# fenghansen/YOND_public

Measured on AMD Instinct MI355X. Metric: Bayer megapixels/sec end-to-end (NLE+VST+denoise+iVST), higher is better.
Workload: dtype f32 (3x3 convolutions: f32 operands as two f16 halves -- 22-23 significant bits -- on the f16 MFMA, 3 products per f32 product, f32 accumulate; per-layer error vs float64 asserted <= 2x the f32 direct kernel's and <= 2e-5 of max|ref| (tests/test_hip_conv.py; measured 1.3e-6 vs 1.5e-6), whole frame v

## Files before the change

include/yond_hip.h:

```cpp
#ifndef YOND_HIP_H
#define YOND_HIP_H

#include <stddef.h>
#include <stdint.h>

#ifdef __cplusplus
extern "C" {
#endif

#define YOND_OK 0
#define YOND_EINVAL (-1)
#define YOND_EUNSUPPORTED (-2)

#define YOND_ABI_VERSION 8
int yond_abi_version(void);

int yond_pack_vst_norm_f32(const float* bayer, int H, int W, float* out, int pad_l, int pad_r, int pad_t,
                           int pad_b, int mode, double scale, double gain, double sigma, double lo,
                           double hi, const double* lut_x, const float* lut_y, int lut_n, float* img_max,
                           void* stream);

int yond_pack_vst_norm_biaslut_f32(const float* bayer, int H, int W, float* out, int pad_l, int pad_r, int pad_t,
                                   int pad_b, double scale, double gain, double sigma, double lo, double hi,
                                   const double* lut_x, const double* lut_y, int lut_n, float* img_max, void* stream);
// ... 28 lines not shown
typedef struct YondConvDesc {
    const float* src0;
    const float* src1;
    int C0, C1;
    int N, H, W;
    int Ho, Wo;
    int Cout;
    int ksize;
    int stride;
    int shuffle;
    int pre_act;
    int post_act;
    float slope;
    const float* wpk;
    const float* escale;
    const float* eshift;
    int ebatch;
    const float* res;
    float* dst;
    int tn;
    int kc;
    int algo;
    const float* out4_w;
    const float* out4_b;
    const float* out4_x;
    const float* out4_ub;
    float* out4_dst;
    unsigned int* status;
    int in_fmt, out_fmt;
    int res_fmt;
    unsigned long long* clk;
    int tile_order;
    float* dst2;
} YondConvDesc;
#define YOND_STATUS_HALF_OVERFLOW 1u
#define YOND_FMT_NHWC_F32 0
#define YOND_FMT_SPLIT_PLANES 1
#define YOND_FMT_PLANES4 2
#define YOND_SP_PLANE_UNITS(H, W) ((((H) * (W)) + 8) / 8 * 8)
#define YOND_SP_BYTES(N, C, H, W) ((size_t)(N) * ((C) / 16) * 4 * (size_t)YOND_SP_PLANE_UNITS(H, W) * 16)
#define YOND_HP_BYTES(N, C, H, W) ((size_t)(N) * ((C) / 16) * 2 * (size_t)YOND_SP_PLANE_UNITS(H, W) * 16)

int yond_conv_config(int ksize, int stride, int cin, int cout, int shuffle, int N, int Ho, int Wo, int* tn, int* kc);
int yond_pack_conv_weight_f32(const float* w, int cout, int cin, int ksize, int tn, int kc, float* dst);
int yond_pack_conv_weight_split_f32(const float* w, int cout, int cin, int ksize, int tn, int kc, float* dst);
int yond_conv2d_f32(const YondConvDesc* desc, void* stream);

int yond_conv_wino_supported(int cin, int cout);
int yond_pack_conv_wino_weight_f32(const float* w, int cout, int cin, int tn, float* dst);

int yond_conv_split_supported(int ksize, int stride, int cin, int cout);
int yond_pack_conv_split_weight_f32(const float* w, int cout, int cin, int ksize, int tn, int parts, float* dst);
int yond_gemm_k1_stationary_supported(const YondConvDesc* desc);
int yond_pack_conv_split_weight_dev_f32(const float* w, int cout, int cin, int ksize, int tn, int parts, float* dst, int* status,
                                        void* stream);
int yond_pack_conv_split_weights_batch_dev_f32(const float* src, const long long* desc, int nlayers, float* dst, size_t ngroups,
                                               int* status, void* stream);

int yond_conv_in_f32(const float* x, const float* ub , int N, int H, int W, int Cout,
                     const float* wpk, const float* bias, float slope, float* dst,
                     int out_fmt , void* stream);
int yond_pack_conv_in_weight_f32(const float* w , int cout, float* dst );

int yond_conv_out_f32(const float* feat , int Cin, const float* w ,
                      const float* bias , const float* x ,
                      const float* ub , int N, int H, int W, float* dst ,
                      void* stream);

int yond_maxpool2_f32(const float* src, int N, int H, int W, int C, float* dst, void* stream);

typedef struct YondFilmDesc {
    int kind, C, ld;
    const float *w_a0, *b_a0, *w_a2, *b_a2;
    const float *w_b0, *b_b0;
    const float *w_b, *b_b;
    const float *cb1, *cb2;
    float *s1, *t1, *s2, *t2;
} YondFilmDesc;
int yond_film_f32(const YondFilmDesc* descs, int nblocks, const float* t , const float* ub ,
                  int N, void* stream);

int yond_box_stats_self1_f32(const float* bayer, int H, int W, int k, int k2, int tile_w, float* mean,
                             float* var, float* blur2, void* stream);
int yond_box_stats_self2_f32(const float* blur2, int h, int w, int k, int tile_w, float* lap, void* stream);
int yond_box_stats_collab_f32(const float* bayer_lr, const float* bayer_hr, int H, int W, int k, int tile_w,
                              float* mean, float* var, float* lap, void* stream);


int yond_box_stats_self_stats_f32(const float* bayer, int H, int W, int k, int k2, int tile_w, float* mean, float* var,
                                  float* blur2, float* lap, const double* q_host, int nq, void* ws, void* stream);
int yond_box_stats_collab_stats_f32(const float* bayer_lr, const float* bayer_hr, int H, int W, int k, int tile_w,
                                    float* mean, float* var, float* lap, const double* q_host, int nq, void* ws, void* stream);

size_t yond_select_ws_bytes(int nr);
int yond_select_ranks_f32(const float* data, size_t n, const int64_t* ranks_host, int nr, float* out, void* ws,
                          void* stream);
int yond_percentiles_f32(const float* data, size_t n, const double* q_host, int nq, double* out, void* ws,
                         void* stream);

size_t yond_nle_ws_bytes(size_t n);
int yond_nle_stats_f32(const float* lap, const float* mean, size_t n, int width, const double* q_host, int nq, void* ws,
                       void* stream);
int yond_nle_threshold_f32(const float* lap, size_t n, const double* q_host, int nq, int want_score, void* ws, void* stream);
int yond_nle_state_layout(int* off );
int yond_nle_moments_f32(const float* lap, const float* mean, const float* var, size_t n, void* ws, void* stream);

// ... 214 lines not shown
```

yond_public_amd/_lib.py:

```python
import ctypes as C
import os

import torch

_HERE = os.path.dirname(os.path.abspath(__file__))
LIB_PATH = os.environ.get("YOND_HIP_LIB", os.path.join(_HERE, "libyond_hip.so"))
_lib = None
ABI_VERSION = 8

vp, i32, f32, f64, sz, i64 = C.c_void_p, C.c_int, C.c_float, C.c_double, C.c_size_t, C.c_longlong


class YondConvDesc(C.Structure):
    _fields_ = [("src0", vp), ("src1", vp), ("C0", i32), ("C1", i32), ("N", i32), ("H", i32), ("W", i32),
                ("Ho", i32), ("Wo", i32), ("Cout", i32), ("ksize", i32), ("stride", i32), ("shuffle", i32),
                ("pre_act", i32), ("post_act", i32), ("slope", f32), ("wpk", vp), ("escale", vp),
                ("eshift", vp), ("ebatch", i32), ("res", vp), ("dst", vp), ("tn", i32), ("kc", i32), ("algo", i32),
                ("out4_w", vp), ("out4_b", vp), ("out4_x", vp), ("out4_ub", vp), ("out4_dst", vp), ("status", vp),
                ("in_fmt", i32), ("out_fmt", i32), ("res_fmt", i32), ("clk", vp), ("tile_order", i32), ("dst2", vp)]


class YondBlock0Desc(C.Structure):
    _fields_ = [("x", vp), ("in_fmt", i32), ("N", i32), ("H", i32), ("W", i32), ("w1", vp), ("w2", vp),
                ("s1", vp), ("t1", vp), ("s2", vp), ("t2", vp), ("ebatch", i32), ("dst", vp),
                ("out4_w", vp), ("out4_b", vp), ("out4_x", vp), ("out4_ub", vp), ("out4_dst", vp), ("status", vp)]


class YondFilmDesc(C.Structure):
    _fields_ = [("kind", i32), ("C", i32), ("ld", i32),
                ("w_a0", vp), ("b_a0", vp), ("w_a2", vp), ("b_a2", vp), ("w_b0", vp), ("b_b0", vp),
                ("w_b", vp), ("b_b", vp), ("cb1", vp), ("cb2", vp),
                ("s1", vp), ("t1", vp), ("s2", vp), ("t2", vp)]


PROTOTYPES = {
    "yond_abi_version": [],
    "yond_pack_vst_norm_f32": [vp, i32, i32, vp, i32, i32, i32, i32, i32, f64, f64, f64, f64, f64, vp, vp, i32, vp, vp],
    "yond_pack_vst_norm_biaslut_f32": [vp, i32, i32, vp, i32, i32, i32, i32, f64, f64, f64, f64, f64, vp, vp, i32, vp, vp],
    "yond_bias_eval_f32": [vp, sz, vp, vp, i32, i32, i32, f64, f64, vp, vp],
    "yond_denorm_ivst_unpack_f32": [vp, i32, i32, i32, i32, i32, i32, vp, i32, f64, f64, f64, f64, f64, i32, vp],
    "yond_pack_vst_norm_batch_f32": [vp, i32, i32, i32, vp, i32, i32, i32, i32, f64, f64, f64, f64, f64, vp, vp, i32, i32, vp, vp],
    "yond_denorm_ivst_unpack_batch_f32": [vp, i32, i32, i32, i32, i32, i32, i32, vp, i32, f64, f64, f64, f64, f64, i32, vp],
    "yond_vst_elem_f32": [vp, sz, f64, f64, f64, vp, vp],
    "yond_ivst_elem_f64": [vp, sz, f64, f64, i32, vp, vp],
    "yond_bayer2rggb_f32": [vp, i32, i32, vp, vp],
    "yond_rggb2bayer_f32": [vp, i32, i32, vp, vp],
    "yond_rot90_f32": [vp, i32, i32, i32, i32, vp, vp],
    "yond_nchw4_to_nhwc4_f32": [vp, vp, i32, i32, i32, vp],
    "yond_nhwc4_to_nchw4_f32": [vp, vp, i32, i32, i32, vp],
    "yond_image_max_f32": [vp, i32, sz, vp, vp, vp],
    "yond_conv_config": [i32, i32, i32, i32, i32, i32, i32, i32, C.POINTER(i32), C.POINTER(i32)],
    "yond_pack_conv_weight_f32": [vp, i32, i32, i32, i32, i32, vp],
    "yond_conv2d_f32": [C.POINTER(YondConvDesc), vp],
    "yond_conv_wino_supported": [i32, i32],
    "yond_pack_conv_wino_weight_f32": [vp, i32, i32, i32, vp],
    "yond_pack_conv_weight_split_f32": [vp, i32, i32, i32, i32, i32, vp],
    "yond_conv_split_supported": [i32, i32, i32, i32],
    "yond_pack_conv_split_weight_f32": [vp, i32, i32, i32, i32, i32, vp],
    "yond_gemm_k1_stationary_supported": [C.POINTER(YondConvDesc)],
    "yond_pack_conv_split_weight_dev_f32": [vp, i32, i32, i32, i32, i32, vp, vp, vp],
    "yond_pack_conv_split_weights_batch_dev_f32": [vp, vp, i32, vp, sz, vp, vp],
    "yond_conv_in_f32": [vp, vp, i32, i32, i32, i32, vp, vp, f32, vp, i32, vp],
    "yond_pack_conv_in_weight_f32": [vp, i32, vp],
    "yond_conv_out_f32": [vp, i32, vp, vp, vp, vp, i32, i32, i32, vp, vp],
    "yond_maxpool2_f32": [vp, i32, i32, i32, i32, vp, vp],
    "yond_film_f32": [vp, i32, vp, vp, i32, vp],
    "yond_box_stats_self1_f32": [vp, i32, i32, i32, i32, i32, vp, vp, vp, vp],
    "yond_box_stats_self2_f32": [vp, i32, i32, i32, i32, vp, vp],
    "yond_box_stats_collab_f32": [vp, vp, i32, i32, i32, i32, vp, vp, vp, vp],
    "yond_box_stats_self_stats_f32": [vp, i32, i32, i32, i32, i32, vp, vp, vp, vp, vp, i32, vp, vp],
    "yond_box_stats_collab_stats_f32": [vp, vp, i32, i32, i32, i32, vp, vp, vp, vp, i32, vp, vp],
    "yond_select_ws_bytes": [i32],
    "yond_select_ranks_f32": [vp, sz, vp, i32, vp, vp, vp],
    "yond_percentiles_f32": [vp, sz, vp, i32, vp, vp, vp],
    "yond_nle_ws_bytes": [sz],
    "yond_nle_stats_f32": [vp, vp, sz, i32, vp, i32, vp, vp],
    "yond_nle_threshold_f32": [vp, sz, vp, i32, i32, vp, vp],
    "yond_nle_state_layout": [vp],
    "yond_nle_moments_f32": [vp, vp, vp, sz, vp, vp],
    "yond_nlf_occupancy_f32": [vp, vp, sz, i32, vp, i32, vp, vp],
    "yond_nlf_score3_f64": [vp, vp, vp, i32, vp, vp, vp],
    "yond_nlf_moments_f32": [vp, vp, vp, sz, vp, vp, vp],
    "yond_bias_lut_f64": [vp, i32, f64, f64, vp, vp],
    "yond_block_metrics_tiles": [i32, i32],
    "yond_block_metrics_f32": [vp, vp, i32, i32, i32, i32, vp, vp],
    "yond_block_metrics_rgb8": [vp, vp, i32, i32, i32, i32, vp, vp],
    "yond_render_srgb": [vp, i32, i32, i32, i32, i32, C.POINTER(f64), C.POINTER(f64), i32, vp, vp, i32, vp, f64, vp],
    "yond_clock_probe": [f64, vp, vp],
    "yond_img2raw_f32": [vp, sz, i32, i32, i32, vp, vp, i32, i32, i32, vp, vp, vp, vp],
    "yond_pg_noise_f32": [vp, vp, sz, i32, vp, i32, vp],
    "yond_camera_noise_f32": [vp, vp, sz, i32, vp, i32, i32, vp],
    "yond_est_conv_in_f32": [vp, i32, i32, i32, i32, vp, vp, vp, vp],
    "yond_est_head_f32": [vp, i32, i32, i32, i32, vp, vp, i32, i32, i32, vp, vp, vp],
    "yond_est_head_ws_bytes": [i32, i32],
    "yond_conv_wgrad_f32": [vp, vp, i32, i32, i32, i32, i32, i32, i32, i32, i32, vp, vp],
    "yond_conv_wgrad_ws_f32": [vp, vp, i32, i32, i32, i32, i32, i32, i32, i32, i32, vp, vp, sz, vp],
    "yond_conv_wgrad_ws_bytes": [i32, i32, i32, i32, i32, i32, i32, i32, i32],
    "yond_conv_wgrad_split_ws_bytes": [i32, i32, i32, i32, i32],
    "yond_conv_wgrad_split_f32": [vp, vp, i32, i32, i32, i32, i32, vp, i32, vp, sz, vp, vp],
    "yond_colsum_f32": [vp, sz, i32, vp, vp],
    "yond_film_silu_supported": [i32],
    "yond_film_silu_f32": [vp, vp, vp, vp, i32, sz, i32, vp],
    "yond_film_silu_bwd_f32": [vp, vp, vp, vp, vp, vp, vp, i32, sz, i32, vp],
    "yond_film_mlp_fwd_f32": [vp, vp, vp, vp, vp, vp, vp, i32, i32, i32, vp, vp, vp],
    "yond_film_mlp_bwd_f32": [vp, vp, vp, vp, vp, vp, vp, vp, i32, i32, i32, vp, vp, vp, vp, vp, vp, vp, vp],
    "yond_film_mlp_fwd_multi_f32": [vp, i32, vp],
    "yond_gemm_split_f32": [vp, i32, sz, i32, i32, i64, i64, i32, vp, vp, i32, i32, i32, i32, vp, vp],
    "yond_film_mlp_bwd_multi_f32": [vp, i32, vp],
    "yond_silu_bwd_add_f32": [vp, vp, vp, vp, sz, vp],
    "yond_silu_f32": [vp, vp, sz, vp],
    "yond_zero_interleave_f32": [vp, i32, i32, i32, i32, i32, i32, vp, vp],
    "yond_l1_loss_f32": [vp, vp, sz, vp, vp, vp],
# ... 113 lines not shown
```

yond_public_amd/csrc/conv.hip:

```cpp
#include "common.h"
#include <cstdlib>

#ifndef YOND_B32_WGS
#define YOND_B32_WGS 2
#endif
#ifndef YOND_ABL
#define YOND_ABL 0
#endif

template <int KS, int STRIDE, int TH, int TN, int KC>
struct ConvCfg {
    static constexpr int TW = 32;
    static constexpr int TAPS = KS * KS;
    static constexpr int PADK = KS / 2;
    static constexpr int IH = (TH - 1) * STRIDE + KS;
    static constexpr int IW = (TW - 1) * STRIDE + KS;
    static constexpr int HALF = (IW + 1) / 2;
    static constexpr int TWP = (STRIDE == 2) ? 2 * HALF : IW;
    static constexpr int PS = KC + 4;
    static constexpr int IN_FLOATS = IH * TWP * PS;
    static constexpr int Q = KC / 8;
    static constexpr int W_FLOATS = TAPS * Q * 2 * TN * 4;
    static constexpr int BUF_FLOATS = IN_FLOATS + W_FLOATS;
    static constexpr int NW = TN / 32;
// ... 467 lines not shown
    {
        const long e11 = yond_exp_long("YOND_1X1_TN", 0), es2 = yond_exp_long("YOND_S2_TN", 0), ekc = yond_exp_long("YOND_CONV_KC", 0),
                   etn = yond_exp_long("YOND_CONV_TN", 0);
        if (e11 && ksize == 1) t = e11 == 32 ? 32 : (ntile % 64 == 0 ? 64 : 32);
        if (es2 && ksize == 3 && stride == 2) t = es2 == 32 ? 32 : (ntile % 64 == 0 ? 64 : 32);
        if (ekc && ksize == 3 && stride == 1) k = ekc == 8 ? 8 : 16;
        if (etn && ksize == 3 && stride == 1 && ntile % 64 == 0) t = etn == 32 ? 32 : 64;
    }
#endif
    if (tn) *tn = t;
    if (kc) *kc = k;
    return YOND_OK;
}

extern "C" int yond_pack_conv_weight_f32(const float* w, int cout, int cin, int ksize, int tn, int kc, float* dst) {
    if (!w || !dst || (tn != 32 && tn != 64) || cout % tn != 0 || cin % kc != 0 || kc % 8 != 0) return YOND_EINVAL;
    const int taps = ksize * ksize, Q = kc / 8;
    size_t o = 0;
    for (int ct = 0; ct < cout / tn; ++ct)
        for (int ch = 0; ch < cin / kc; ++ch)
            for (int tap = 0; tap < taps; ++tap)
                for (int q = 0; q < Q; ++q)
                    for (int h = 0; h < 2; ++h)
                        for (int j = 0; j < tn; ++j)
                            for (int e = 0; e < 4; ++e) {
                                const int co = ct * tn + j, ci = ch * kc + q * 8 + h * 4 + e;
                                dst[o++] = w[((size_t)co * cin + ci) * taps + tap];
                            }
    return YOND_OK;
}

extern "C" int yond_pack_conv_weight_split_f32(const float* w, int cout, int cin, int ksize, int tn, int kc, float* dst) {
    const int rc = yond_pack_conv_weight_f32(w, cout, cin, ksize, tn, kc, dst);
    if (rc != YOND_OK) return rc;
    const size_t n = (size_t)cout * cin * ksize * ksize;
    for (size_t i = 0; i < n; ++i)
        if (!(fabsf(w[i]) <= 65504.0f)) return YOND_EUNSUPPORTED;
    for (size_t i = 0; i < n; ++i) {
        const float v = dst[i];
        const _Float16 h = (_Float16)v;
        const _Float16 l = (_Float16)((v - (float)h) * 2048.0f);
        unsigned short hb, lb;
        __builtin_memcpy(&hb, &h, 2);
        __builtin_memcpy(&lb, &l, 2);
        const unsigned u = (unsigned)hb | ((unsigned)lb << 16);
        __builtin_memcpy(&dst[i], &u, 4);
    }
    return YOND_OK;
}

int yond_conv_wino_dispatch(const YondConvDesc& d, hipStream_t st);
int yond_conv_split_dispatch(const YondConvDesc& d, hipStream_t st);
int yond_gemm_k1_stationary_dispatch(const YondConvDesc& d, hipStream_t st);

extern "C" int yond_conv2d_f32(const YondConvDesc* dp, void* stream) {
    if (!dp) return YOND_EINVAL;
    const YondConvDesc& d = *dp;
    hipStream_t st = (hipStream_t)stream;
    if (!d.src0 || !(d.dst || d.out4_dst) || !d.wpk || d.N <= 0 || d.H <= 0 || d.W <= 0 || d.Ho <= 0 || d.Wo <= 0) return YOND_EINVAL;
    if (d.out4_dst && ((d.algo != 3 && d.algo != 4) || !d.out4_w || d.Cout != 32 || d.stride != 1)) return YOND_EUNSUPPORTED;
    if (d.C1 > 0 && !d.src1) return YOND_EINVAL;
    if (d.shuffle < 0 || d.shuffle > 2) return YOND_EINVAL;
    if (d.shuffle == 2 && d.algo != 3 && d.algo != 4 && d.algo != 6) return YOND_EUNSUPPORTED;
    if ((long long)d.N * d.H * d.W > 0x7fffffffLL) return YOND_EUNSUPPORTED;
    if (d.pre_act != 0 && d.pre_act != 1) return YOND_EINVAL;
    if (d.in_fmt < 0 || d.in_fmt > 2 || d.out_fmt < 0 || d.out_fmt > 2 || (d.res_fmt != 0 && d.res_fmt != 2)) return YOND_EINVAL;
    if (d.algo == 6) return yond_gemm_k1_stationary_dispatch(d, st);
    if ((d.in_fmt || d.out_fmt || d.res_fmt) && d.algo != 3 && d.algo != 4) return YOND_EUNSUPPORTED;
    if (d.algo == 1) return yond_conv_wino_dispatch(d, st);
    if (d.algo == 3 || d.algo == 4) return yond_conv_split_dispatch(d, st);
    if (d.algo != 0 && d.algo != 2 && d.algo != 5) return YOND_EINVAL;
    if (d.tn != 32 && d.tn != 64) return YOND_EINVAL;
    int tn, kc;
    const int rc = yond_conv_config(d.ksize, d.stride, d.C0 + d.C1, d.Cout, d.shuffle, 0, 0, 0, &tn, &kc);
    if (rc != YOND_OK) return rc;
    tn = d.tn;
    if (d.kc != 0) kc = d.kc;
    if (kc != 8 && kc != 16) return YOND_EINVAL;
    if (kc == 8 && d.ksize != 3) return YOND_EINVAL;
    if (d.ksize == 3 && d.stride == 2 && kc != 8) return YOND_EINVAL;
    if (d.C0 % kc != 0 || d.C1 % kc != 0 || d.Cout % tn != 0) return YOND_EUNSUPPORTED;
    if (d.shuffle && (d.ksize != 1 || (d.Cout / 4) % tn != 0)) return YOND_EUNSUPPORTED;
    if ((long long)d.N * d.H * d.W > 0x7fffffffLL) return YOND_EUNSUPPORTED;
    if (d.stride == 2) {
        if (d.Ho != (d.H + 1) / 2 || d.Wo != (d.W + 1) / 2) return YOND_EINVAL;
    } else if (d.Ho != d.H || d.Wo != d.W) return YOND_EINVAL;
    if (d.pre_act != 0 && d.pre_act != 1) return YOND_EINVAL;
    if (d.post_act != 0 && d.post_act != 2) return YOND_EUNSUPPORTED;
    if (d.pre_act == 1 && !(d.ksize == 3 && d.stride == 1)) return YOND_EUNSUPPORTED;
    if (d.ksize == 3 && d.stride == 1 && kc == 8) {
        if (d.pre_act) return tn == 64 ? launch_conv<3, 1, 8, 64, 8, true>(d, st) : launch_conv<3, 1, 8, 32, 8, true>(d, st);
        return tn == 64 ? launch_conv<3, 1, 8, 64, 8, false>(d, st) : launch_conv<3, 1, 8, 32, 8, false>(d, st);
    }
    if (d.ksize == 3 && d.stride == 1) {
        if (d.pre_act) return tn == 64 ? launch_conv<3, 1, 8, 64, 16, true>(d, st) : launch_conv<3, 1, 8, 32, 16, true>(d, st);
        return tn == 64 ? launch_conv<3, 1, 8, 64, 16, false>(d, st) : launch_conv<3, 1, 8, 32, 16, false>(d, st);
    }
    if (d.ksize == 3 && d.stride == 2)
        return tn == 64 ? launch_conv<3, 2, 8, 64, 8, false>(d, st) : launch_conv<3, 2, 4, 32, 8, false>(d, st);
    return tn == 64 ? launch_conv<1, 1, 8, 64, 16, false>(d, st) : launch_conv<1, 1, 8, 32, 16, false>(d, st);
}
```

yond_public_amd/engine.py:

```python
import ctypes as C
import os

import numpy as np
import torch

from . import _lib as L


def _rup(c, m=32):
    return (c + m - 1) // m * m


def _np_ptr(a):
    return C.c_void_p(a.ctypes.data)


FILM_MAX_C = 1024


WINO_DEFAULT = 'split'


SPLIT_PLANES = True
SP_FLOW = True
HALF_FLOW = True
HALF_K1_TN128 = True
HALF_S2_TN128 = True
HALF_FLOW_TN128 = True
HALF_TN128 = True
FUSE_OUT4 = True
FUSE_BLOCK0 = False
K1_SUB2 = True
K1_D2_LEVELS = (3,)
K1_STATIONARY_LEVELS = (2, 1, 0)
K1_D2_LEVELS_HALF = ()
SP_CONV1_MIN_LEVEL = 3
UNET_SP = True
SNAKE_ORDER = True


def sp_plane_units(H, W):
    return (H * W + 8) // 8 * 8


class _PackedConv:

    def __init__(self, dev, weight, bias, ksize, stride, splits, shuffle=False):
        lib = L.load()
        w = weight.detach().to('cpu', torch.float32).numpy()
        if shuffle:
            cin, cout = w.shape[0], w.shape[1]
            coutp = _rup(cout)
            m = np.zeros((4, coutp, cin), np.float32)
            m[:, :cout, :] = w.transpose(2, 3, 1, 0).reshape(4, cout, cin)
            w = m.reshape(4 * coutp, cin, 1, 1)
            self.cout_real_p = coutp
            gemm_n = 4 * coutp
        else:
            cout = w.shape[0]
            coutp = _rup(cout)
            gemm_n = coutp
            self.cout_real_p = coutp
        assert sum(splits) == w.shape[1], (splits, w.shape)
        psplits = [_rup(s) for s in splits]
        cinp = sum(psplits)
        wp = np.zeros((gemm_n, cinp, ksize, ksize), np.float32)
        so, do = 0, 0
        for s, ps in zip(splits, psplits):
            wp[:w.shape[0], do:do + s] = w[:, so:so + s]
            so += s
            do += ps
        self._wp = np.ascontiguousarray(wp)
        self._packed = {}
        self._dev = dev
        b = torch.zeros(coutp, dtype=torch.float32)
        if bias is not None:
            b[:cout] = bias.detach().to('cpu', torch.float32)
        self.bias = b.to(dev)
        self.ksize, self.stride, self.shuffle = ksize, stride, shuffle
        self.psplits, self.gemm_n, self.coutp, self.cinp = psplits, gemm_n, coutp, cinp
        self.cin_real, self.cout_real = sum(splits), cout
        self.config(0, 0, 0)
        self.wmax = float(np.abs(self._wp).max()) if self._wp.size else 0.0
        self.macs_per_pixel = self.cin_real * self.cout_real * (4 if shuffle else ksize * ksize)

    def config(self, N, Ho, Wo, split=False):
        lib = L.load()
# ... 239 lines not shown
        d.ksize, d.stride, d.shuffle = pc.ksize, pc.stride, int(pc.shuffle)
        d.pre_act, d.post_act, d.slope = pre_act, post_act, slope
        prec = getattr(self, 'precision', 'fp32')
        if getattr(self, 'strict', False) and algo is None:
            prec, algo = 'fp32-mfma', 1
        if algo is None:
            algo = getattr(self, 'conv_algo', WINO_DEFAULT)
            if prec == 'fp32-mfma' and algo == 'split':
                algo = 1
            if prec == 'fp16' and WINO_DEFAULT == 'split':
                algo = 'half'
        fp16 = prec == 'fp16' or algo == 'fp16'
        wino = split = None
        if algo in ('split', 'half'):
            ws2 = (HALF_S2_TN128 and algo == 'half' and pc.stride == 2 and in_fmt == 1 and out_fmt == 2 and dst2 is None
                   and (pc.gemm_n // 128) * ((d.Wo + 31) // 32) * ((d.Ho + 7) // 8) * N >= 256)
            ws2 = ws2 or (HALF_K1_TN128 and algo == 'half' and pc.ksize == 1 and in_fmt == 1 and dst2 is None)
            split = pc.split(2 if algo == 'split' else 1, wide=(not (in_fmt or out_fmt or res_fmt or dst2 is not None)) or (HALF_FLOW_TN128 and out_fmt == 1),
                             wide_s2=ws2)
            if algo == 'half' and pc.ksize == 1 and in_fmt != 1:
                split = None
            if split is None and not fp16 and pc.ksize == 3:
                wino = pc.wino()
        elif not fp16:
            wino = pc.wino() if algo in (1, 2) else None
        if split is not None:
            tn, wpk = split
            kc = 16
            d.algo = 3 if algo == 'split' else 4
        elif wino is not None:
            tn, wpk = wino
            kc = 8
            d.algo = 1
        elif algo == 'split' and pc.ksize == 1 and not fp16 and pc.config(N, d.Ho, d.Wo, split=True)[2] is not None:
            tn, kc, wpk = pc.config(N, d.Ho, d.Wo, split=True)
            d.algo = 5
        else:
            tn, kc, wpk = pc.config(N, d.Ho, d.Wo)
            d.algo = 2 if (fp16 and pc.wmax <= 65504.0) else 0
        d.wpk = wpk.data_ptr()
        d.tn = tn
        d.kc = kc
        d.escale = escale.data_ptr() if escale is not None else None
        d.eshift = (eshift if eshift is not None else pc.bias).data_ptr()
        d.ebatch = ebatch
        d.res = res.data_ptr() if res is not None else None
        d.dst = dst.data_ptr() if dst is not None else None
        status = getattr(self, 'status', None)
        d.status = status.data_ptr() + 4 * self.status_slot if status is not None else None
        d.in_fmt, d.out_fmt, d.res_fmt = in_fmt, out_fmt, res_fmt
        d.dst2 = dst2.data_ptr() if dst2 is not None else None
        if stationary and d.algo == 3 and self.lib.yond_gemm_k1_stationary_supported(C.byref(d)):
            d.algo = 6
        if SNAKE_ORDER and d.algo in (3, 4, 6):
            self._tile_order = 1 - getattr(self, '_tile_order', 0)
            d.tile_order = self._tile_order
        clk = getattr(self, 'clk', None)
        d.clk = clk.data_ptr() if (clk is not None and d.algo in (3, 4, 6)) else None
        if (in_fmt or out_fmt or res_fmt) and d.algo not in (3, 4, 6):
            raise L.YondHipError("split-plane / 4-channel-plane tensors need the split-operand kernel (algo 3, or 4 with h-only planes)")
        if out4 is not None:
            w4, b4, x4, ub4, o4 = out4
            if d.algo not in (3, 4):
                raise L.YondHipError("fused output projection needs the split-operand 3x3 kernel")
            d.out4_w, d.out4_b = w4.data_ptr(), (b4.data_ptr() if b4 is not None else None)
            d.out4_x = x4.data_ptr() if x4 is not None else None
            d.out4_ub = ub4.data_ptr() if ub4 is not None else None
            d.out4_dst = o4.data_ptr()
        prof = getattr(self, 'prof', None)
        if prof is not None:
            tag = f"conv_wino_kernel<{tn}>" if d.algo == 1 else f"conv_mfma_kernel<{pc.ksize},{pc.stride},8,{tn},{kc}>"
            if d.algo in (3, 4, 6):
                tag = f"conv_split_kernel<{pc.stride if pc.ksize == 3 else 'k1'},{tn},{1 if d.algo == 4 else 2}>" + ("/stationary" if d.algo == 6 else "")
            if d.algo == 2:
                tag += "/f16"
            if d.algo == 5:
                tag += "/split"
            only = getattr(self, 'prof_only', None)
            if only is not None and not only(tag):
                prof = None
            every = getattr(self, 'prof_every', 1)
            if every > 1 and getattr(self, '_fwd_idx', 0) % every:
                prof = None
        if prof is not None:
            e0, e1 = torch.cuda.Event(enable_timing=True), torch.cuda.Event(enable_timing=True)
            e0.record()
        L.check(self.lib.yond_conv2d_f32(C.byref(d), L.stream()), "yond_conv2d_f32")
        if prof is not None:
            e1.record()
            prof.append((tag, 2.0 * pc.macs_per_pixel * N * d.Ho * d.Wo, e0, e1))
        return dst

    def _block0_weights(self, pc):
        w = getattr(pc, '_b0', None)
        if w is None:
            if not L.has("yond_pack_block0_weight_f32"):
                raise L.YondHipError("the fused level-0 block exists only in experiment builds of the library (python -m yond_public_amd.build --experiments)")
            if not (pc.ksize == 3 and pc.stride == 1 and pc.gemm_n == 32 and pc.cinp == 32 and len(pc.psplits) == 1):
                return None
            host = np.zeros(9 * 2 * 4 * 32 * 8, np.float16)
            if self.lib.yond_pack_block0_weight_f32(_np_ptr(pc._wp), 32, 32, _np_ptr(host)) != 0:
                return None
            w = pc._b0 = torch.from_numpy(host.view(np.float32)).to(pc._dev)
        return w

    def _block0(self, pc1, pc2, x, N, H, W, f, in_fmt, dst=None, out4=None):
        w1, w2 = self._block0_weights(pc1), self._block0_weights(pc2)
        d = L.YondBlock0Desc()
        d.x, d.in_fmt, d.N, d.H, d.W = x.data_ptr(), in_fmt, N, H, W
        d.w1, d.w2 = w1.data_ptr(), w2.data_ptr()
        d.s1, d.t1, d.s2, d.t2 = (None if v is None else v.data_ptr() for v in f)
        d.ebatch = 1
        d.dst = dst.data_ptr() if dst is not None else None
        if out4 is not None:
            w4, b4, x4, ub4, o4 = out4
            d.out4_w, d.out4_b = w4.data_ptr(), (b4.data_ptr() if b4 is not None else None)
            d.out4_x = x4.data_ptr() if x4 is not None else None
            d.out4_ub = ub4.data_ptr() if ub4 is not None else None
            d.out4_dst = o4.data_ptr()
        status = getattr(self, 'status', None)
        d.status = status.data_ptr() + 4 * self.status_slot if status is not None else None
        prof = getattr(self, 'prof', None)
        if prof is not None:
            tag = "block0_fused_kernel" + ("<o4>" if out4 is not None else "")
            only = getattr(self, 'prof_only', None)
            if (only is not None and not only(tag)) or (getattr(self, 'prof_every', 1) > 1 and getattr(self, '_fwd_idx', 0) % getattr(self, 'prof_every', 1)):
# ... 67 lines not shown
        self._fwd_idx = getattr(self, '_fwd_idx', -1) + 1
        self._tile_order = 0
        N, H, W, c4 = x4.shape
        if c4 != 4 or H % 16 or W % 16:
            raise L.YondHipError(f"input must be [N][H][W][4] with H, W multiples of 16, got {tuple(x4.shape)}")
        if self.norm and ub is None:
            ub = self.image_max(x4, N)
        if not self.norm:
            ub = None
        st = L.stream()
        lib = self.lib
        nfp = _rup(self.nf)
        if self.guided:
            if t_dev is None:
                raise L.YondHipError(f"{self.kind}.forward needs the noise level t")
            film = self._film(t_dev, ub, N)
            flow = self._sp_flow(N, H, W)
            pt = 1 if (flow and getattr(self, 'precision', 'fp32') == 'fp16') else 2
            P4, SP = 2, 1
            a = self._new(N, H, W, nfp)
            L.check(lib.yond_conv_in_f32(L.ptr(x4), L.ptr(ub), N, H, W, nfp, L.ptr(self.conv_in_w), L.ptr(self.conv_in_b),
                                         0.01, L.ptr(a), P4 if flow else 0, st), "yond_conv_in_f32")
            skips = {}
            h, w = H, W
            cur = a
            xsp = None
            for i in range(1, 10):
                blk = self.blocks[i]
                cp = blk['Cp']
                f = film[f'conv{i}']
                last = i == 9
                xfmt = P4 if (flow and not last) else 0
                if i >= 6:
                    xs = self._new(N, 2 * h, 2 * w, cp)
                    up = blk['upsc2'] if (flow and K1_SUB2 and 'upsc2' in blk) else blk['upsc']
                    xsp = (self._new_sp(('xspd', i), N, 2 * h, 2 * w, cp, pt)
                           if (flow and not last and (9 - i) in (K1_D2_LEVELS if pt == 2 else K1_D2_LEVELS_HALF) and up is blk['upsc'] and cp % 64 == 0 and w > 16) else None)
                    self._conv(up, cur, skips[10 - i], N, h, w, xs, in_fmt=SP if flow else 0, out_fmt=xfmt, dst2=xsp,
                               stationary=(9 - i) in K1_STATIONARY_LEVELS)
                    h, w = 2 * h, 2 * w
                    cur = xs
                if flow and FUSE_BLOCK0 and h == H and cp == 32 and self._block0_weights(blk['conv1']) is not None and self._block0_weights(blk['conv2']) is not None:
                    if last and self._out4_fusable(blk['conv2'], flow):
                        out4 = self._new(N, H, W, 4)
                        self._block0(blk['conv1'], blk['conv2'], cur, N, h, w, f, xfmt, out4=(self.w_out, self.b_out, x4 if self.res else None, ub, out4))
                        return out4
                    if not last:
                        out = self._new_sp(('out', i), N, h, w, cp, pt)
                        self._block0(blk['conv1'], blk['conv2'], cur, N, h, w, f, xfmt, dst=out)
                        cur = out
                        skips[i] = cur
                        nxt = self._new(N, h // 2, w // 2, blk['pool'].coutp)
                        xsp = self._new_sp(('xsp', i + 1), N, h // 2, w // 2, blk['pool'].coutp, pt) if (flow and i >= SP_CONV1_MIN_LEVEL) else None
                        self._conv(blk['pool'], cur, None, N, h, w, nxt, in_fmt=SP, out_fmt=P4, dst2=xsp)
                        h, w = h // 2, w // 2
                        cur = nxt
                        continue
                act_in_producer = self._split_pair(blk['conv1'], blk['conv2'])
                sp = SP if (flow or (act_in_producer and SPLIT_PLANES and getattr(self, 'precision', 'fp32') == 'fp32'
                                      and sp_plane_units(h, w) * 64 < 2 ** 31)) else 0
                tmp = self._new_sp(('tmp', i), N, h, w, cp, pt) if sp else self._new(N, h, w, cp)
                if xsp is not None and sp and act_in_producer:
                    self._conv(blk['conv1'], xsp, None, N, h, w, tmp, escale=f[0], eshift=f[1], ebatch=1, pre_act=0, post_act=1,
                               in_fmt=SP, out_fmt=sp)
                else:
                    self._conv(blk['conv1'], cur, None, N, h, w, tmp, escale=f[0], eshift=f[1], ebatch=1, pre_act=1,
                               post_act=1 if act_in_producer else 0, in_fmt=xfmt, out_fmt=sp)
                xsp = None
                pre2 = 0 if act_in_producer else 1
                if last and self._out4_fusable(blk['conv2'], flow):
                    out4 = self._new(N, H, W, 4)
                    self._conv(blk['conv2'], tmp, None, N, h, w, None, escale=f[2], eshift=f[3], ebatch=1, res=cur, pre_act=pre2,
                               out4=(self.w_out, self.b_out, x4 if self.res else None, ub, out4), in_fmt=sp)
                    return out4
                if flow:
                    out = self._new_sp(('out', i), N, h, w, cp, pt)
                    self._conv(blk['conv2'], tmp, None, N, h, w, out, escale=f[2], eshift=f[3], ebatch=1, res=cur, pre_act=pre2,
                               in_fmt=SP, out_fmt=SP, res_fmt=P4)
                else:
                    out = self._new(N, h, w, cp)
                    self._conv(blk['conv2'], tmp, None, N, h, w, out, escale=f[2], eshift=f[3], ebatch=1, res=cur, pre_act=pre2, in_fmt=sp)
                cur = out
                if i <= 4:
                    skips[i] = cur
                    nxt = self._new(N, h // 2, w // 2, blk['pool'].coutp)
                    xsp = self._new_sp(('xsp', i + 1), N, h // 2, w // 2, blk['pool'].coutp, pt) if (flow and i >= SP_CONV1_MIN_LEVEL) else None
                    self._conv(blk['pool'], cur, None, N, h, w, nxt, in_fmt=SP if flow else 0, out_fmt=P4 if flow else 0, dst2=xsp)
                    h, w = h // 2, w // 2
                    cur = nxt
            feat = cur
        else:
            a = self._new(N, H, W, nfp)
            L.check(lib.yond_conv_in_f32(L.ptr(x4), L.ptr(ub), N, H, W, nfp, L.ptr(self.conv_in_w), L.ptr(self.conv_in_b),
                                         0.2, L.ptr(a), 0, st), "yond_conv_in_f32")
            cv = self.convs
            h, w = H, W
            cur = self._conv(cv['conv1_2'], a, None, N, h, w, self._new(N, h, w, cv['conv1_2'].coutp), post_act=2, slope=0.2)
            skips = {1: cur}

            def first_of_pair(i, c1, c2, s0, s1):
                sp = (UNET_SP and SPLIT_PLANES and not getattr(self, 'strict', False) and getattr(self, 'conv_algo', WINO_DEFAULT) == 'split'
                      and getattr(self, 'precision', 'fp32') == 'fp32' and c1.split(2) is not None and c2.split(2) is not None
                      and N * sp_plane_units(h, w) * 64 < 2 ** 31)
                dst = self._new_sp(('utmp', i), N, h, w, c1.coutp) if sp else self._new(N, h, w, c1.coutp)
                self._conv(c1, s0, s1, N, h, w, dst, post_act=2, slope=0.2, out_fmt=1 if sp else 0)
                return dst, (1 if sp else 0)

            for i in range(2, 6):
                cpv = cur.shape[-1]
                pooled = self._new(N, h // 2, w // 2, cpv)
                L.check(lib.yond_maxpool2_f32(L.ptr(cur), N, h, w, cpv, L.ptr(pooled), st), "yond_maxpool2_f32")
                h, w = h // 2, w // 2
                c1, c2 = cv[f'conv{i}_1'], cv[f'conv{i}_2']
                cur, fmt = first_of_pair(i, c1, c2, pooled, None)
                cur = self._conv(c2, cur, None, N, h, w, self._new(N, h, w, c2.coutp), post_act=2, slope=0.2, in_fmt=fmt)
                if i < 5:
                    skips[i] = cur
            for i in range(6, 10):
                upc = cv[f'upv{i}']
                up = self._new(N, 2 * h, 2 * w, upc.cout_real_p)
                self._conv(upc, cur, None, N, h, w, up)
                h, w = 2 * h, 2 * w
                c1, c2 = cv[f'conv{i}_1'], cv[f'conv{i}_2']
                cur, fmt = first_of_pair(i, c1, c2, up, skips[10 - i])
                if i == 9 and self._out4_fusable(c2):
                    out4 = self._new(N, H, W, 4)
                    self._conv(c2, cur, None, N, h, w, None, post_act=2, slope=0.2, in_fmt=fmt,
                               out4=(self.w_out, self.b_out, x4 if self.res else None, ub, out4))
                    return out4
                cur = self._conv(c2, cur, None, N, h, w, self._new(N, h, w, c2.coutp), post_act=2, slope=0.2, in_fmt=fmt)
            feat = cur
        out4 = self._new(N, H, W, 4)
        L.check(lib.yond_conv_out_f32(L.ptr(feat), feat.shape[-1], L.ptr(self.w_out), L.ptr(self.b_out),
                                      L.ptr(x4) if self.res else None, L.ptr(ub), N, H, W, L.ptr(out4), st), "yond_conv_out_f32")
        return out4

    def forward_nchw(self, x, t=None):
        L.require_cuda(x, "x")
        N, c, H, W = x.shape
        if c != 4:
# ... 28 lines not shown
```

Measured before the change: 2673.

## Add weight-stationary persistent kernel for stride-2 3x3 downsampling conv

Adds a new persistent kernel (algo 7) for the stride-2 3x3 pool convolutions. It keeps the full 64-output-channel weight slice in LDS for the whole kernel and streams 32-pixel row segments through a register ring of prefetched split-f16 input loads. It is enabled for N==1 at level 1 only, where xsp/dst2 is None. The aim is to cut repeated weight reloads and tile overheads of the generic split kernel for this layer. In exchange it adds a large specialised code path with a fixed grid, high register pressure and narrow applicability.

```diff
diff --git a/include/yond_hip.h b/include/yond_hip.h
--- a/include/yond_hip.h
+++ b/include/yond_hip.h
@@ -104,6 +104,7 @@
 int yond_conv_split_supported(int ksize, int stride, int cin, int cout);
 int yond_pack_conv_split_weight_f32(const float* w, int cout, int cin, int ksize, int tn, int parts, float* dst);
 int yond_gemm_k1_stationary_supported(const YondConvDesc* desc);
+int yond_conv_s2_stationary_supported(const YondConvDesc* desc);
 int yond_pack_conv_split_weight_dev_f32(const float* w, int cout, int cin, int ksize, int tn, int parts, float* dst, int* status,
                                         void* stream);
 int yond_pack_conv_split_weights_batch_dev_f32(const float* src, const long long* desc, int nlayers, float* dst, size_t ngroups,
diff --git a/yond_public_amd/_lib.py b/yond_public_amd/_lib.py
--- a/yond_public_amd/_lib.py
+++ b/yond_public_amd/_lib.py
@@ -58,6 +58,7 @@
     "yond_conv_split_supported": [i32, i32, i32, i32],
     "yond_pack_conv_split_weight_f32": [vp, i32, i32, i32, i32, i32, vp],
     "yond_gemm_k1_stationary_supported": [C.POINTER(YondConvDesc)],
+    "yond_conv_s2_stationary_supported": [C.POINTER(YondConvDesc)],
     "yond_pack_conv_split_weight_dev_f32": [vp, i32, i32, i32, i32, i32, vp, vp, vp],
     "yond_pack_conv_split_weights_batch_dev_f32": [vp, vp, i32, vp, sz, vp, vp],
     "yond_conv_in_f32": [vp, vp, i32, i32, i32, i32, vp, vp, f32, vp, i32, vp],
diff --git a/yond_public_amd/csrc/conv.hip b/yond_public_amd/csrc/conv.hip
--- a/yond_public_amd/csrc/conv.hip
+++ b/yond_public_amd/csrc/conv.hip
@@ -543,6 +543,7 @@
 int yond_conv_wino_dispatch(const YondConvDesc& d, hipStream_t st);
 int yond_conv_split_dispatch(const YondConvDesc& d, hipStream_t st);
 int yond_gemm_k1_stationary_dispatch(const YondConvDesc& d, hipStream_t st);
+int yond_conv_s2_stationary_dispatch(const YondConvDesc& d, hipStream_t st);
 
 extern "C" int yond_conv2d_f32(const YondConvDesc* dp, void* stream) {
     if (!dp) return YOND_EINVAL;
@@ -557,6 +558,7 @@
     if (d.pre_act != 0 && d.pre_act != 1) return YOND_EINVAL;
     if (d.in_fmt < 0 || d.in_fmt > 2 || d.out_fmt < 0 || d.out_fmt > 2 || (d.res_fmt != 0 && d.res_fmt != 2)) return YOND_EINVAL;
     if (d.algo == 6) return yond_gemm_k1_stationary_dispatch(d, st);
+    if (d.algo == 7) return yond_conv_s2_stationary_dispatch(d, st);
     if ((d.in_fmt || d.out_fmt || d.res_fmt) && d.algo != 3 && d.algo != 4) return YOND_EUNSUPPORTED;
     if (d.algo == 1) return yond_conv_wino_dispatch(d, st);
     if (d.algo == 3 || d.algo == 4) return yond_conv_split_dispatch(d, st);
diff --git a/yond_public_amd/csrc/conv_s2_stationary.hip b/yond_public_amd/csrc/conv_s2_stationary.hip
--- /dev/null
+++ b/yond_public_amd/csrc/conv_s2_stationary.hip
@@ -0,0 +1,223 @@
+#include "common.h"
+
+typedef _Float16 f16x8 __attribute__((ext_vector_type(8)));
+typedef unsigned u32x4 __attribute__((ext_vector_type(4)));
+
+template <int NCH, int D, bool ROWS = false>
+__global__ __launch_bounds__(512) void conv_s2_stationary_kernel(const YondConvDesc d) {
+    constexpr int NST = NCH * 9;
+    constexpr int TNK = 64, NW = 2;
+    constexpr int WS = 2;
+    static_assert(NST % D == 0 && NST % WS == 0 && D >= 2, "the ring holds whole rounds of a segment's steps");
+    static_assert(!ROWS || (D == 9 && NCH % 2 == 0), "row-by-row refill: one chunk in the ring, the slot rotation closes at the segment's end");
+    constexpr int W_FLOATS = NST * 4 * TNK * 4;
+    constexpr int FILM_OFF = W_FLOATS;
+    extern __shared__ __attribute__((aligned(16))) float smem[];
+    const int tid = threadIdx.x, lane = tid & 63, wave = __builtin_amdgcn_readfirstlane(tid >> 6);
+    const int li = lane & 31, lh = lane >> 5;
+    const int nct = d.Cout / TNK;
+    const int per_xcd = gridDim.x / 8;
+    const int bx = blockIdx.x % 8, bj = blockIdx.x / 8;
+    const int ct = bj % nct, gj = bj / nct, G = per_xcd / nct;
+    const bool clk_on = d.clk != nullptr && blockIdx.x == 0 && tid == 0;
+    unsigned long long clk_c0 = 0, clk_r0 = 0;
+    if (clk_on) { clk_c0 = __builtin_amdgcn_s_memtime(); clk_r0 = __builtin_amdgcn_s_memrealtime(); }
+
+    {
+        f32x4* wl = (f32x4*)smem;
+        const f32x4* wsrc = (const f32x4*)(d.wpk + (size_t)ct * W_FLOATS);
+        for (int i = tid; i < NST * 4 * 64; i += 512) wl[i] = wsrc[i];
+        float* film = smem + FILM_OFF;
+        const int nfilm = d.ebatch ? d.N : 1;
+        for (int i = tid; i < nfilm * 2 * TNK; i += 512) {
+            const int im = i / (2 * TNK), k = i % (2 * TNK);
+            const int cb = ct * TNK + (k % TNK);
+            film[i] = k < TNK ? (d.escale ? d.escale[im * d.Cout + cb] : 1.0f) : (d.eshift ? d.eshift[im * d.Cout + cb] : 0.0f);
+        }
+    }
+    __syncthreads();
+
+    const int H = d.H, W = d.W, Ho = d.Ho, Wo = d.Wo;
+    const int nsx = (Wo + 31) / 32;
+    const int nseg = d.N * Ho * nsx;
+    const int lo = (int)((long long)nseg * bx / 8), hi = (int)((long long)nseg * (bx + 1) / 8);
+    const int sstep = 8 * G;
+    const int s0 = lo + gj + G * wave;
+    if (s0 < hi) {
+        const bool rev = d.tile_order != 0;
+        const size_t PS = (size_t)YOND_SP_PLANE_UNITS(H, W) * 16;
+        const float slope_eff = d.post_act == 2 ? d.slope : 1.0f;
+        struct Geo { int n, y, x; unsigned v[9]; };
+        auto geo = [&](int s) {
+            Geo g;
+            const int t = rev ? nseg - 1 - s : s;
+            const int per = Ho * nsx;
+            g.n = t / per;
+            const int r = t - g.n * per;
+            g.y = r / nsx;
+            g.x = (r - g.y * nsx) * 32 + li;
+            const bool in = g.x < Wo;
+            const unsigned hb = (unsigned)((size_t)lh * 2 * PS);
+#pragma unroll
+            for (int dy = 0; dy < 3; ++dy) {
+                const int iy = 2 * g.y + dy - 1;
+                const bool rok = in && iy >= 0 && iy < H;
+#pragma unroll
+                for (int dx = 0; dx < 3; ++dx) {
+                    const int ix = 2 * g.x + dx - 1;
+                    const bool ok = rok && ix >= 0 && ix < W;
+                    g.v[dy * 3 + dx] = hb + (unsigned)(ok ? iy * W + ix : H * W) * 16u;
+                }
+            }
+            return g;
+        };
+        f16x8 ring[D][2];
+        auto issue = [&](auto tc, const Geo& g) __attribute__((always_inline)) {
+            constexpr int t = decltype(tc)::value, c = t / 9, k = t % 9;
+            constexpr int dx = ROWS ? k % 3 : k / 3, dy = ROWS ? k / 3 : k % 3;
+            constexpr int slot = ROWS ? ((c & 1) ? dy * 3 + dx : dx * 3 + dy) : t % D;
+            const char* b = (const char*)d.src0 + (size_t)g.n * NCH * 4 * PS;
+            ring[slot][0] = *(const f16x8*)(b + (g.v[dy * 3 + dx] + (unsigned)(c * 4) * (unsigned)PS));
+            ring[slot][1] = *(const f16x8*)(b + (g.v[dy * 3 + dx] + (unsigned)(c * 4 + 1) * (unsigned)PS));
+        };
+        typedef const __attribute__((address_space(3))) f16x8* lds_h8;
+        unsigned wb[3];
+#pragma unroll
+        for (int i = 0; i < 3; ++i) {
+            wb[i] = (unsigned)(uintptr_t)(__attribute__((address_space(3))) float*)(smem + (lh * 2 * TNK + li) * 4) + (unsigned)i * 65536u;
+            asm volatile("" : "+v"(wb[i]));
+        }
+        const float* film = smem + FILM_OFF;
+        const unsigned hw_out = (unsigned)(Ho * Wo);
+        const __amdgpu_buffer_rsrc_t orsrc = __builtin_amdgcn_make_buffer_rsrc(d.dst, 0, (int)((unsigned)d.N * (unsigned)d.Cout * hw_out * 4u), 0x00020000);
+        f16x8 wt[WS][NW][2];
+        auto load_w = [&](auto sc) __attribute__((always_inline)) {
+            constexpr int s = decltype(sc)::value;
+            constexpr int c = s / 9, q = s % 9, dx = q / 3, dy = q % 3, tap = c * 9 + dy * 3 + dx;
+#pragma unroll
+            for (int nn = 0; nn < NW; ++nn)
+#pragma unroll
+                for (int p = 0; p < 2; ++p) {
+                    const int off = ((tap * 4 + p) * TNK + nn * 32) * 16;
+                    wt[s % WS][nn][p] = *(lds_h8)(uintptr_t)(wb[off >> 16] + (unsigned)(off & 0xffff));
+                }
+        };
+
+        auto segment = [&](const Geo& cur, Geo& nxt, int sg) __attribute__((always_inline)) {
+            f32x16 acc[2][NW];
+#pragma unroll
+            for (int a = 0; a < 2; ++a)
+#pragma unroll
+                for (int nn = 0; nn < NW; ++nn)
+#pragma unroll
+                    for (int r = 0; r < 16; ++r) acc[a][nn][r] = 0.0f;
+            static_for<0, NST>([&](auto sc) __attribute__((always_inline)) {
+                constexpr int s = decltype(sc)::value, ws = s % WS;
+                constexpr int slot = ROWS ? (((s / 9) & 1) ? (s % 3) * 3 + (s % 9) / 3 : s % 9) : s % D;
+                load_w(IntC<(s + 1) % NST>{});
+                const f16x8 xh = ring[slot][0], xl = ring[slot][1];
+#pragma unroll
+                for (int nn = 0; nn < NW; ++nn) acc[1][nn] = __builtin_amdgcn_mfma_f32_32x32x16_f16(wt[ws][nn][0], xl, acc[1][nn], 0, 0, 0);
+#pragma unroll
+                for (int nn = 0; nn < NW; ++nn) acc[0][nn] = __builtin_amdgcn_mfma_f32_32x32x16_f16(wt[ws][nn][0], xh, acc[0][nn], 0, 0, 0);
+#pragma unroll
+                for (int nn = 0; nn < NW; ++nn) acc[1][nn] = __builtin_amdgcn_mfma_f32_32x32x16_f16(wt[ws][nn][1], xh, acc[1][nn], 0, 0, 0);
+                if constexpr (s + D < NST) issue(IntC<s + D>{}, cur);
+                else issue(IntC<s + D - NST>{}, nxt);
+                if constexpr (s + D + 1 == NST) nxt = geo(sg);
+                __builtin_amdgcn_sched_barrier(0);
+            });
+            const unsigned pixo = (unsigned)(cur.y * Wo + cur.x);
+            const unsigned mask = cur.x < Wo ? 0u : 0x80000000u;
+            const float* fv = film + (d.ebatch ? cur.n * 2 * TNK : 0) + 4 * lh;
+#pragma unroll
+            for (int nn = 0; nn < NW; ++nn) {
+                const int cbase = ct * TNK + nn * 32 + 4 * lh;
+                const unsigned ob = (((unsigned)(cur.n * (d.Cout / 4) + cbase / 4) * hw_out + pixo) * 16u) | mask;
+#pragma unroll
+                for (int g = 0; g < 4; ++g) {
+                    const f32x4 es = *(const f32x4*)(fv + nn * 32 + 8 * g), et = *(const f32x4*)(fv + TNK + nn * 32 + 8 * g);
+                    f32x4 v;
+#pragma unroll
+                    for (int e = 0; e < 4; ++e) {
+                        float x = acc[0][nn][4 * g + e];
+                        x = fmaf(acc[1][nn][4 * g + e], 1.0f / 2048.0f, x);
+                        x = fmaf(x, es[e], et[e]);
+                        x = x > 0.0f ? x : x * slope_eff;
+                        v[e] = x + 0.0f;
+                    }
+                    __builtin_amdgcn_raw_buffer_store_b128(__builtin_bit_cast(u32x4, v), orsrc, (int)(ob + (unsigned)g * 32u * hw_out), 0, 0);
+                }
+            }
+        };
+
+        int sc = s0;
+        Geo cur = geo(sc), nxt;
+        static_for<0, D>([&](auto kc) { issue(kc, cur); });
+        load_w(IntC<0>{});
+        int sn = sc + sstep;
+        segment(cur, nxt, sn < hi ? sn : sc);
+        while (sn < hi) {
+            cur = nxt;
+            sc = sn;
+            sn += sstep;
+            segment(cur, nxt, sn < hi ? sn : sc);
+        }
+        asm volatile("s_waitcnt vmcnt(0)" ::: "memory");
+    }
+    if (clk_on) {
+        atomicAdd(d.clk, __builtin_amdgcn_s_memtime() - clk_c0);
+        atomicAdd(d.clk + 1, __builtin_amdgcn_s_memrealtime() - clk_r0);
+    }
+}
+
+static int s2s_chunks(const YondConvDesc& d) {
+    if (d.ksize != 3 || d.stride != 2 || d.shuffle != 0 || d.tn != 64 || !d.src0 || d.src1 || d.C1 || !d.dst || !d.wpk) return 0;
+    if (d.in_fmt != YOND_FMT_SPLIT_PLANES || d.out_fmt != YOND_FMT_PLANES4 || d.res_fmt || d.res || d.dst2 || d.out4_dst || d.pre_act) return 0;
+    if (d.post_act != 0 && d.post_act != 2) return 0;
+    if (d.N <= 0 || d.H <= 0 || d.W <= 0 || d.Ho != (d.H + 1) / 2 || d.Wo != (d.W + 1) / 2 || d.Cout <= 0 || d.Cout % 64) return 0;
+    const int nch = d.C0 == 32 ? 2 : d.C0 == 64 ? 4 : 0;
+    if (!nch) return 0;
+    const int nct = d.Cout / 64;
+    if (nct > 32 || 32 % nct) return 0;
+    if (d.ebatch && d.N > 16) return 0;
+    if ((long long)d.N * d.H * d.W > 0x7fffffffLL) return 0;
+    if ((long long)d.N * d.Ho * ((d.Wo + 31) / 32 * 32) > 0x7fffffffLL) return 0;
+    if ((long long)d.N * d.Cout * d.Ho * d.Wo * 4 >= 0x7fffffffLL) return 0;
+    if ((long long)YOND_SP_PLANE_UNITS(d.H, d.W) * 16 * 4 * nch >= 0x7fffffffLL) return 0;
+    return nch;
+}
+
+extern "C" int yond_conv_s2_stationary_supported(const YondConvDesc* d) { return (d && (d->algo == 3 || d->algo == 7) && s2s_chunks(*d)) ? 1 : 0; }
+
+template <int NCH, int D, bool ROWS = false>
+static int launch_s2s(const YondConvDesc& d, hipStream_t st) {
+    constexpr int SMEM = (NCH * 9 * 4 * 64 * 4 + 16 * 2 * 64) * 4;
+    static_assert(SMEM <= 160 * 1024, "LDS budget");
+    static bool attr_set = false;
+    auto kern = conv_s2_stationary_kernel<NCH, D, ROWS>;
+    if (!attr_set) {
+        hipError_t e = hipFuncSetAttribute((const void*)kern, hipFuncAttributeMaxDynamicSharedMemorySize, SMEM);
+        if (e != hipSuccess) return (int)e;
+        attr_set = true;
+    }
+    constexpr int S2S_GRID = 256;
+    static_assert(S2S_GRID % 8 == 0, "whole XCD shares");
+    hipLaunchKernelGGL(kern, dim3(S2S_GRID), dim3(512), SMEM, st, d);
+    YOND_LAUNCH_CHECK();
+    return YOND_OK;
+}
+
+int yond_conv_s2_stationary_dispatch(const YondConvDesc& d, hipStream_t st) {
+    const int nch = s2s_chunks(d);
+#ifdef YOND_EXPERIMENTS
+    const long depth = yond_exp_long("YOND_S2S_DEPTH", 0);
+    if (nch == 2 && depth == 3) return launch_s2s<2, 3>(d, st);
+    if (nch == 2 && depth == 6) return launch_s2s<2, 6>(d, st);
+    if (nch == 4 && depth == 3) return launch_s2s<4, 3>(d, st);
+    if (nch == 4 && depth == 6) return launch_s2s<4, 6>(d, st);
+#endif
+    if (nch == 2) return launch_s2s<2, 9, true>(d, st);
+    if (nch == 4) return launch_s2s<4, 9, true>(d, st);
+    return YOND_EUNSUPPORTED;
+}
diff --git a/yond_public_amd/engine.py b/yond_public_amd/engine.py
--- a/yond_public_amd/engine.py
+++ b/yond_public_amd/engine.py
@@ -33,6 +33,7 @@
 K1_SUB2 = True
 K1_D2_LEVELS = (3,)
 K1_STATIONARY_LEVELS = (2, 1, 0)
+S2_STATIONARY_LEVELS = (1,)
 K1_D2_LEVELS_HALF = ()
 SP_CONV1_MIN_LEVEL = 3
 UNET_SP = True
@@ -378,12 +379,14 @@
         d.dst2 = dst2.data_ptr() if dst2 is not None else None
         if stationary and d.algo == 3 and self.lib.yond_gemm_k1_stationary_supported(C.byref(d)):
             d.algo = 6
-        if SNAKE_ORDER and d.algo in (3, 4, 6):
+        elif stationary and d.algo == 3 and self.lib.yond_conv_s2_stationary_supported(C.byref(d)):
+            d.algo = 7
+        if SNAKE_ORDER and d.algo in (3, 4, 6, 7):
             self._tile_order = 1 - getattr(self, '_tile_order', 0)
             d.tile_order = self._tile_order
         clk = getattr(self, 'clk', None)
-        d.clk = clk.data_ptr() if (clk is not None and d.algo in (3, 4, 6)) else None
-        if (in_fmt or out_fmt or res_fmt) and d.algo not in (3, 4, 6):
+        d.clk = clk.data_ptr() if (clk is not None and d.algo in (3, 4, 6, 7)) else None
+        if (in_fmt or out_fmt or res_fmt) and d.algo not in (3, 4, 6, 7):
             raise L.YondHipError("split-plane / 4-channel-plane tensors need the split-operand kernel (algo 3, or 4 with h-only planes)")
         if out4 is not None:
             w4, b4, x4, ub4, o4 = out4
@@ -396,8 +399,8 @@
         prof = getattr(self, 'prof', None)
         if prof is not None:
             tag = f"conv_wino_kernel<{tn}>" if d.algo == 1 else f"conv_mfma_kernel<{pc.ksize},{pc.stride},8,{tn},{kc}>"
-            if d.algo in (3, 4, 6):
-                tag = f"conv_split_kernel<{pc.stride if pc.ksize == 3 else 'k1'},{tn},{1 if d.algo == 4 else 2}>" + ("/stationary" if d.algo == 6 else "")
+            if d.algo in (3, 4, 6, 7):
+                tag = f"conv_split_kernel<{pc.stride if pc.ksize == 3 else 'k1'},{tn},{1 if d.algo == 4 else 2}>" + ("/stationary" if d.algo == 6 else "/stationary-s2" if d.algo == 7 else "")
             if d.algo == 2:
                 tag += "/f16"
             if d.algo == 5:
@@ -571,7 +574,7 @@
                         skips[i] = cur
                         nxt = self._new(N, h // 2, w // 2, blk['pool'].coutp)
                         xsp = self._new_sp(('xsp', i + 1), N, h // 2, w // 2, blk['pool'].coutp, pt) if (flow and i >= SP_CONV1_MIN_LEVEL) else None
-                        self._conv(blk['pool'], cur, None, N, h, w, nxt, in_fmt=SP, out_fmt=P4, dst2=xsp)
+                        self._conv(blk['pool'], cur, None, N, h, w, nxt, in_fmt=SP, out_fmt=P4, dst2=xsp, stationary=N == 1 and (i - 1) in S2_STATIONARY_LEVELS)
                         h, w = h // 2, w // 2
                         cur = nxt
                         continue
@@ -604,7 +607,8 @@
                     skips[i] = cur
                     nxt = self._new(N, h // 2, w // 2, blk['pool'].coutp)
                     xsp = self._new_sp(('xsp', i + 1), N, h // 2, w // 2, blk['pool'].coutp, pt) if (flow and i >= SP_CONV1_MIN_LEVEL) else None
-                    self._conv(blk['pool'], cur, None, N, h, w, nxt, in_fmt=SP if flow else 0, out_fmt=P4 if flow else 0, dst2=xsp)
+                    self._conv(blk['pool'], cur, None, N, h, w, nxt, in_fmt=SP if flow else 0, out_fmt=P4 if flow else 0, dst2=xsp,
+                               stationary=N == 1 and (i - 1) in S2_STATIONARY_LEVELS)
                     h, w = h // 2, w // 2
                     cur = nxt
             feat = cur
```

Result: no change. 2695 (median of 6 runs) (+0.8%).
